# chaiyujin/sdfa-2019

Measured on AMD Instinct MI355X. Metric: animation frames/s/node (10 s@16 kHz clips); max|Δdgrad| vs CPU ref, higher is better.
Workload: dtype f32

## Files before the change

sdfa-2019_amd/csrc/api_core.cpp:

```cpp
#include "../../include/sdfa_stream.h"
#include "host.h"

#include <climits>
#include <cstdio>
#include <cstring>
#include <string>

static thread_local std::string g_err;

int sdfa_failv(int code, const char *fmt, va_list ap) {
    char buf[512];
    vsnprintf(buf, sizeof buf, fmt, ap);
    g_err = buf;
    return code;
}

int sdfa_fail(int code, const char *fmt, ...) {
    va_list ap;
    va_start(ap, fmt);
    sdfa_failv(code, fmt, ap);
    va_end(ap);
    return code;
}

thread_local int g_sdfa_mel_fft_radix4 = 0;
thread_local int g_sdfa_gather_plain_order = 0;
thread_local int g_sdfa_frontend_two_kernel = 0;
thread_local int g_sdfa_frontend_stream_block = 0;
thread_local int g_sdfa_frontend_stream_slots = 0;
thread_local int g_sdfa_frontend_stream_spin_max = 0;
thread_local int g_sdfa_frontend_stream_phases = 0;
thread_local int g_sdfa_frontend_t_major = 0;
extern thread_local int g_sdfa_gemm_variant;
thread_local int g_sdfa_freq_lstm_shape = 0;
thread_local int g_sdfa_pca_lds = 0;
thread_local int g_sdfa_pca_fp32 = 0;
thread_local int g_sdfa_conv_fp32 = 0;
thread_local int g_sdfa_time_lstm_split = 0;
thread_local int g_sdfa_time_lstm_handoff = 0;
thread_local int g_sdfa_time_lstm_timeout_us = 0;
thread_local int g_sdfa_share_gx0_off = 0;
thread_local int g_sdfa_encoder_dedup_off = 0;
thread_local int g_sdfa_freq_proj_tail = 0;
thread_local int g_sdfa_attn_unfused = 0;

extern "C" {

int sdfa_abi_version(void) { return SDFA_ABI_VERSION; }
int sdfa_stream_abi_version(void) { return SDFA_STREAM_ABI_VERSION; }
const char *sdfa_last_error(void) { return g_err.c_str(); }

int sdfa_debug_set_option(const char *name, int value) {
    struct Option { const char *name; int *var; int lo = INT_MIN, hi = INT_MAX; const char *accepts = nullptr; };
    thread_local const Option options[] = {
        {"attn_unfused", &g_sdfa_attn_unfused},
        {"share_gx0_off", &g_sdfa_share_gx0_off},
        {"encoder_dedup_off", &g_sdfa_encoder_dedup_off},
        {"freq_proj_tail", &g_sdfa_freq_proj_tail, 0, 2, "0 (rule), 1 (never) or 2 (always)"},
        {"frontend_two_kernel", &g_sdfa_frontend_two_kernel},
        {"frontend_stream_phases", &g_sdfa_frontend_stream_phases},
        {"frontend_stream_spin_max", &g_sdfa_frontend_stream_spin_max, 0, INT_MAX, "0 (default) or a positive poll count"},
        {"frontend_stream_block", &g_sdfa_frontend_stream_block, 0, 256, "0 (default) or 1..256 frames"},
        {"frontend_stream_slots", &g_sdfa_frontend_stream_slots, 0, 256, "0 (default) or 1..256 workgroups per block"},
        {"gather_plain_order", &g_sdfa_gather_plain_order},
        {"mel_fft_radix4", &g_sdfa_mel_fft_radix4},
        {"frontend_t_major", &g_sdfa_frontend_t_major},
        {"time_lstm_timeout_us", &g_sdfa_time_lstm_timeout_us},
        {"time_lstm_handoff", &g_sdfa_time_lstm_handoff},
        {"time_lstm_split", &g_sdfa_time_lstm_split},
        {"gemm_variant", &g_sdfa_gemm_variant},
        {"freq_lstm_shape", &g_sdfa_freq_lstm_shape},
        {"pca_lds", &g_sdfa_pca_lds},
        {"conv_fp32", &g_sdfa_conv_fp32},
        {"pca_fp32", &g_sdfa_pca_fp32},
    };
    for (const Option &o : options)
        if (name && !strcmp(name, o.name)) {
            if (value < o.lo || value > o.hi) return sdfa_fail(SDFA_EINVAL, "%s: %s", o.name, o.accepts);
            *o.var = value;
            return SDFA_OK;
        }
    return sdfa_fail(SDFA_EINVAL, "unknown option '%s'", name ? name : "(null)");
}

}
```

sdfa-2019_amd/csrc/api_forward.cpp:

```cpp
#include "common.h"
#include "host.h"
#include "kernels.h"
#include "model.h"

#include <algorithm>

extern thread_local int g_sdfa_gemm_variant, g_sdfa_freq_lstm_shape, g_sdfa_pca_lds, g_sdfa_pca_fp32, g_sdfa_conv_fp32, g_sdfa_share_gx0_off, g_sdfa_attn_unfused, g_sdfa_encoder_dedup_off,
    g_sdfa_freq_proj_tail;

namespace {

constexpr int64_t CT_WORDS = 2048, CT_FLAGS = 16, ST_WORDS = SDFA_WS_STATUS_BYTES / 4;

struct Ws {
    int64_t P1, X3, HF, Z, GX, H0, H1, KP, QC, QP, ZK, SH, ZU, total;
    int64_t TRUNK, A0, A1, COEF;
    int64_t CT_FREQ, CT_PCA, CT_FLAG;
};

Ws layout(int64_t Nc, bool keep) {
    const int64_t Mc = 64 * Nc;
    Ws w{};
    int64_t o = 0;
    auto take = [&](int64_t n) { int64_t r = o; o += round_up(n, 64); return r; };
    take(ST_WORDS);
    if (keep) {
        w.P1 = take(2048 * Mc); w.X3 = take(2048 * Mc); w.HF = take((int64_t)HF_SLAB_ROWS * 4 * Mc); w.Z = take(256 * Mc);
        w.GX = take(2048 * Mc); w.H0 = take(512 * Mc); w.H1 = take(512 * Mc); w.KP = take(128 * Mc);
    } else {
        const int64_t A = take(2048 * Mc);
        const int64_t B = take(2048 * Mc);
        w.HF = take((int64_t)HF_SLAB_ROWS * 4 * Mc);
        w.P1 = A; w.GX = A;
        w.X3 = B; w.Z = B; w.H0 = B + 256 * Mc; w.H1 = B + 768 * Mc; w.KP = B + 1280 * Mc;
    }
    w.QC = take(512 * Nc); w.QP = take(128 * Nc); w.ZK = take(512 * Nc);
    const int64_t R = take(2560 * Nc);
    w.TRUNK = R; w.A0 = R + 512 * Nc; w.A1 = R + 1024 * Nc; w.COEF = R + 1280 * Nc;
    w.SH = take(sdfa_share_table_words(Nc) + 111);
    w.ZU = keep ? take(256 * Mc) : w.P1;
    const int64_t CT = take(CT_WORDS);
    w.CT_FREQ = CT; w.CT_PCA = CT + 1; w.CT_FLAG = CT + CT_FLAGS;
    w.total = o;
    return w;
}

int64_t capacity(int64_t bytes, bool keep) {
    const int64_t per128 = layout(128, keep).total * 4;
    int64_t nc = (bytes / per128 + 2) * 128;
    while (nc > 0 && layout(nc, keep).total * 4 > bytes) nc -= 128;
    return nc;
}

struct Prof {
    const sdfa_model *m;
    hipStream_t s;
    hipEvent_t pending = nullptr;
    void begin(const char *stage) {
        if (!m->profile) return;
        sdfa_model::Ev e; e.stage = stage;
        (void)hipEventCreate(&e.a); (void)hipEventCreate(&e.b);
        (void)hipEventRecord(e.a, s);
        pending = e.b;
        std::lock_guard<std::mutex> lk(m->ev_mu);
        m->events.push_back(e);
    }
    void end() {
        if (!m->profile || !pending) return;
        (void)hipEventRecord(pending, s);
        pending = nullptr;
    }
};

GemmArgs gemm_fc(const sdfa_model::Fc &fc, const float *Q, int64_t ldq, float *D, int64_t Nc, const int64_t *spk, int64_t nreal) {
    GemmArgs g = sdfa_gemm_k4(fc.w, fc.Ppad, Q, ldq, D, Nc, fc.K);
    g.bias = fc.b; g.cond_w = fc.cw; g.cond_idx = fc.cw ? spk : nullptr;
    g.Pstore = fc.Pstore; g.Qreal = nreal; g.act = fc.act;
    return g;
}

}

extern "C" {

int64_t sdfa_workspace_bytes(const sdfa_model *m, int64_t max_frames) {
    if (!m || max_frames <= 0) return sdfa_fail(SDFA_EINVAL, "workspace_bytes: bad argument");
    return layout(round_up(max_frames, 128), m->keep).total * 4;
}

int sdfa_debug_keep_intermediates(sdfa_model *m, int on) {
    if (!m) return sdfa_fail(SDFA_EINVAL, "null model");
    m->keep = on != 0;
    return SDFA_OK;
}

int sdfa_profile_enable(sdfa_model *m, int on) {
    if (!m) return sdfa_fail(SDFA_EINVAL, "null model");
    std::lock_guard<std::mutex> lk(m->ev_mu);
    m->profile = on != 0;
    for (auto &e : m->events) { (void)hipEventDestroy(e.a); (void)hipEventDestroy(e.b); }
    m->events.clear();
    return SDFA_OK;
}

float sdfa_profile_ms(const sdfa_model *m, const char *stage) {
    if (!m || !stage) return (float)sdfa_fail(SDFA_EINVAL, "profile_ms: bad argument");
    float total = 0.f;
    bool any = false;
    std::lock_guard<std::mutex> lk(m->ev_mu);
    for (auto &e : m->events)
        if (e.stage == stage) {
            float ms = 0.f;
            if (hipEventSynchronize(e.b) != hipSuccess || hipEventElapsedTime(&ms, e.a, e.b) != hipSuccess)
                return (float)sdfa_fail(SDFA_EHIP, "profile_ms: event query failed");
            total += ms; any = true;
        }
    return any ? total : (float)sdfa_fail(SDFA_EINVAL, "profile_ms: no such stage '%s'", stage);
}

int sdfa_profile_reset(sdfa_model *m) { return m ? sdfa_profile_enable(m, m->profile) : sdfa_fail(SDFA_EINVAL, "null model"); }

enum { STAGE_BODY = 0, STAGE_ATTENTION = 1, STAGE_REGRESSOR = 2 };
static int stage_terms(const sdfa_model *m, int stage) {
    switch (m->precision) {
    case SDFA_PREC_BF16_ATTENTION: return stage == STAGE_ATTENTION ? 1 : 0;
    case SDFA_PREC_BF16X3_ATTENTION: return stage == STAGE_ATTENTION ? 3 : 0;
    case SDFA_PREC_BF16X6: return 6;
    case SDFA_PREC_BF16X3: return 3;
    case SDFA_PREC_BF16: return 1;
    default: return 0;
    }
}

int sdfa_model_set_precision(sdfa_model *m, int mode) {
    if (!m) return sdfa_fail(SDFA_EINVAL, "null model");
    if (mode < SDFA_PREC_FP32 || mode > SDFA_PREC_BF16X6) return sdfa_fail(SDFA_EINVAL, "unknown precision mode %d", mode);
    m->precision = mode;
    return SDFA_OK;
}

int sdfa_model_precision(const sdfa_model *m) { return m ? m->precision : SDFA_EINVAL; }

int sdfa_model_set_reserved_cus(sdfa_model *m, int k) {
    if (!m) return sdfa_fail(SDFA_EINVAL, "null model");
    if (k < 0 || k > 128) return sdfa_fail(SDFA_EINVAL, "reserved_cus must be in [0, 128], got %d", k);
    m->reserved_cus.store(k);
    return SDFA_OK;
}

static int encoder_impl(const sdfa_model *m, const float *d_audio_feat, int64_t n_frames, const int32_t *d_frame_clip,
                        const int64_t *d_frame_start, int hop, float *d_z, float *d_align, void *d_workspace,
                        int64_t workspace_bytes, void *stream) {
    if (!m || !m->finalized) return sdfa_fail(SDFA_ESTATE, "encoder_forward: model not finalised");
    if (n_frames == 0) return SDFA_OK;
    if (!d_audio_feat || !d_z || !d_workspace || n_frames < 0) return sdfa_fail(SDFA_EINVAL, "encoder_forward: bad argument");
    if (((uintptr_t)d_workspace | (uintptr_t)d_audio_feat | (uintptr_t)d_z) & 15) return sdfa_fail(SDFA_EINVAL, "encoder_forward: pointers must be 16-byte aligned");
    if ((uintptr_t)d_align & 3) return sdfa_fail(SDFA_EINVAL, "encoder_forward: d_align must be 4-byte aligned");
    const int64_t cap = capacity(workspace_bytes, m->keep);
    if (cap < 128) return sdfa_fail(SDFA_ENOSPACE, "encoder_forward: workspace of %lld bytes holds no 128-frame chunk", (long long)workspace_bytes);
    hipStream_t s = (hipStream_t)stream;
    Prof pf{m, s};
    float *ws = (float *)d_workspace;
    for (int64_t f0 = 0; f0 < n_frames; f0 += cap) {
        const int64_t N = std::min(cap, n_frames - f0);
        const int64_t Nc = round_up(N, 128), Mc = 64 * Nc;
        const Ws w = layout(Nc, m->keep);
        ConvArgs ca{};
        ca.audio_feat = d_audio_feat + f0 * (64 * 128 * 3); ca.N = N; ca.Nc = Nc; ca.Mc = Mc;
        ca.w1 = m->w1; ca.b1 = m->b1; ca.s1 = m->s1; ca.t1 = m->t1; ca.P1 = ws + w.P1;
        ca.w2 = m->w2; ca.b2 = m->b2; ca.s2 = m->s2; ca.t2 = m->t2;
        ca.w3 = m->w3; ca.b3 = m->b3; ca.s3 = m->s3; ca.t3 = m->t3; ca.X3 = ws + w.X3;
        const bool table = d_frame_clip != nullptr;
        const bool share = table || (!m->keep && !g_sdfa_encoder_dedup_off);
        const int64_t *d_ulimit = nullptr;
        int32_t *col_to_u = nullptr;
        bool split_tail = false;
        int64_t fat_grid = 0;
        const int64_t *d_qfull = nullptr;
        if (share) {
            ShareArgs sa{};
            sa.N = N; sa.Nc = Nc; sa.Mc = Mc;
            sdfa_share_carve(sa, reinterpret_cast<int32_t *>(ws + w.SH));
            split_tail = !m->keep && stage_terms(m, STAGE_BODY) == 0 && g_sdfa_gemm_variant == 0 && Mc / 256 >= 512 && g_sdfa_freq_proj_tail != 1;
            if (split_tail) {
                fat_grid = sdfa_fat_grid(256, Mc, sdfa_cu_count(), m->reserved_cus.load());
                sa.fat_grid = (int)fat_grid; sa.tail_mode = g_sdfa_freq_proj_tail;
            }
            pf.begin("share_map");
            if (table) {
                sa.frame_clip = d_frame_clip + f0; sa.frame_start = d_frame_start + f0; sa.hop = hop;
                sa.t_lo = 6; sa.t_hi = 58;
                HIP_TRY(sdfa_launch_share_map(sa, s));
            } else {
                sa.feat = ca.audio_feat;
                sa.hash = reinterpret_cast<uint64_t *>(ws + w.HF); sa.linked = sa.hash + Mc;
                HIP_TRY(sdfa_launch_share_map_content(sa, s));
            }
            pf.end();
            d_ulimit = sa.counts + 1; d_qfull = sa.counts + 2; col_to_u = sa.col_to_u;
            ca.col_src = sa.col_src; ca.col_limit = d_ulimit;
        }
        const int conv_terms = g_sdfa_conv_fp32 ? 0 : stage_terms(m, STAGE_BODY);
        if (m->keep && conv_terms) {
            pf.begin("conv1"); HIP_TRY(sdfa_launch_conv1(ca, s)); pf.end();
            ca.wb = m->cv_wb; ca.terms = conv_terms;
            pf.begin("conv23"); HIP_TRY(sdfa_launch_conv123(ca, s)); pf.end();
        } else if (m->keep) {
            pf.begin("conv1"); HIP_TRY(sdfa_launch_conv1(ca, s)); pf.end();
            pf.begin("conv23"); HIP_TRY(sdfa_launch_conv23(ca, s)); pf.end();
        } else {
            ca.wb = m->cv_wb; ca.terms = conv_terms;
            pf.begin("conv23"); HIP_TRY(sdfa_launch_conv123(ca, s)); pf.end();
        }

        const int fl_terms = stage_terms(m, STAGE_BODY);
        FreqLstmArgs fa{ws + w.X3, m->fl_w, m->fl_b, ws + w.HF, Mc, d_ulimit, m->fl_wb, fl_terms, reinterpret_cast<int *>(ws + w.CT_FREQ),
                        g_sdfa_freq_lstm_shape ? g_sdfa_freq_lstm_shape : (fl_terms ? 0 : m->freq_shape.load()), m->reserved_cus.load()};
        pf.begin("freq_lstm"); HIP_TRY(sdfa_launch_freq_lstm(fa, s)); pf.end();

        GemmArgs g = sdfa_gemm_k4(m->fp_w, 256, ws + w.HF, Mc, ws + w.Z, Mc, 8192);
        g.bias = m->fp_b; g.q_tile_major = 1; g.q_slab_rows = HF_SLAB_ROWS;
        g.terms = stage_terms(m, STAGE_BODY);
        g.reserve_cus = m->reserved_cus.load();
        if (share) { g.D = ws + w.ZU; g.q_limit = split_tail ? d_qfull : d_ulimit; }
        pf.begin("freq_proj");
        HIP_TRY(sdfa_launch_gemm(g, s));
        if (split_tail) {
            GemmTailArgs gt{m->fp_w, ws + w.HF, m->fp_b, ws + w.ZU, Mc, HF_SLAB_ROWS, d_qfull, d_ulimit, (int)fat_grid - 1};
            HIP_TRY(sdfa_launch_gemm_tail(gt, s));
        }
        pf.end();
        const bool share_gx0 = share && !m->keep && stage_terms(m, STAGE_BODY) == 0 && !g_sdfa_share_gx0_off;
        if (share && !share_gx0) {
            pf.begin("share_expand"); HIP_TRY(sdfa_launch_expand_cols(ws + w.ZU, col_to_u, ws + w.Z, 64, Mc, s)); pf.end();
        }

        const float *xin = share_gx0 ? ws + w.ZU : ws + w.Z;
        float *hout[2] = {ws + w.H0, ws + w.H1};
        const char *gxn[2] = {"gx0", "gx1"}, *lsn[2] = {"lstm0", "lstm1"};
        for (int l = 0; l < 2; ++l) {
            const bool mapped = share_gx0 && l == 0;
            float *gx = mapped ? ws + w.HF : ws + w.GX;
            GemmArgs gi = sdfa_gemm_k4(m->gx_w[l], 2048, xin, Mc, gx, Mc, l == 0 ? 256 : 512);
            gi.terms = stage_terms(m, STAGE_BODY);
            gi.reserve_cus = m->reserved_cus.load();
            if (mapped) gi.q_limit = d_ulimit;
            pf.begin(gxn[l]); HIP_TRY(sdfa_launch_gemm(gi, s)); pf.end();
            TimeLstmArgs ta{gx, m->tl_w[l], hout[l], Nc, Mc, m->tl_wb[l], stage_terms(m, STAGE_BODY),
                            reinterpret_cast<unsigned *>(ws + w.CT_FLAG), CT_WORDS - CT_FLAGS, m->tl_w16[l],
                            reinterpret_cast<unsigned *>(ws), m->reserved_cus.load(), mapped ? col_to_u : nullptr};
            pf.begin(lsn[l]); HIP_TRY(sdfa_launch_time_lstm(ta, s)); pf.end();
            xin = hout[l];
        }
        const int at_terms = stage_terms(m, STAGE_ATTENTION);
        const bool key_fused = g_sdfa_attn_unfused != 1;
        pf.begin("attn_proj");
        GemmArgs gk = sdfa_gemm_k4(m->kp_w, 128, ws + w.H1, Mc, ws + w.KP, Mc, 512);
        gk.terms = at_terms;
        if (!key_fused) HIP_TRY(sdfa_launch_gemm(gk, s));
        GemmArgs gc = sdfa_gemm_k4(m->qc_w, 512, ws + w.H1 + 31 * Nc * 4, Mc, ws + w.QC, Nc, 1536);
        gc.seg_k = 512; gc.seg_col = Nc; gc.terms = at_terms;
        HIP_TRY(sdfa_launch_gemm(gc, s));
        GemmArgs gq = sdfa_gemm_k4(m->qp_w, 128, ws + w.QC, Nc, ws + w.QP, Nc, 512);
        gq.terms = at_terms;
        HIP_TRY(sdfa_launch_gemm(gq, s));
        const bool tail_fused = key_fused && (at_terms == 0 || at_terms == 6) && g_sdfa_attn_unfused != 2 && sdfa_attn_fuses_tail(Nc, m->reserved_cus.load());
        if (key_fused) {
            AttnKeyArgs ak{};
            ak.Wk = m->kp_w; ak.H = ws + w.H1; ak.QP = ws + w.QP; ak.v = m->at_v; ak.b = m->at_b;
            ak.S = ws + w.KP;
            ak.Nc = Nc; ak.Mc = Mc; ak.terms = at_terms == 6 ? 0 : at_terms; ak.reserve_cus = m->reserved_cus.load();
            if (tail_fused) {
                ak.fuse_tail = 1; ak.Zk4 = ws + w.ZK; ak.z_out = d_z + f0 * 512; ak.align_out = d_align ? d_align + f0 * 64 : nullptr; ak.N = N;
            }
            HIP_TRY(sdfa_launch_attn_key_score(ak, s));
        }
        pf.end();

        AttnArgs aa{};
        aa.KP = ws + w.KP; aa.QP = ws + w.QP; aa.H = ws + w.H1; aa.v = m->at_v; aa.b = m->at_b;
        aa.Zk4 = ws + w.ZK; aa.z_out = d_z + f0 * 512; aa.align_out = d_align ? d_align + f0 * 64 : nullptr;
        aa.N = N; aa.Nc = Nc; aa.Mc = Mc;
        aa.S = key_fused ? ws + w.KP : nullptr;
        pf.begin("attn"); if (!tail_fused) HIP_TRY(sdfa_launch_attn(aa, s)); pf.end();
    }
    return SDFA_OK;
}

int sdfa_model_autotune(sdfa_model *m, int64_t n_frames, void *d_workspace, int64_t workspace_bytes, void *stream) {
    if (!m || !m->finalized) return sdfa_fail(SDFA_ESTATE, "autotune: model not finalised");
    if (!d_workspace || n_frames <= 0 || ((uintptr_t)d_workspace & 15)) return sdfa_fail(SDFA_EINVAL, "autotune: bad argument");
    const int64_t cap = capacity(workspace_bytes, m->keep);
    if (cap < 128) return sdfa_fail(SDFA_ENOSPACE, "autotune: workspace too small");
    const int64_t Nc = round_up(std::min(cap, n_frames), 128), Mc = 64 * Nc;
    const Ws w = layout(Nc, m->keep);
    float *ws = (float *)d_workspace;
    hipStream_t s = (hipStream_t)stream;
    HIP_TRY(hipMemsetAsync(ws + w.X3, 0, (size_t)2048 * Mc * sizeof(float), s));
    hipEvent_t e0, e1;
    HIP_TRY(hipEventCreate(&e0));
    HIP_TRY(hipEventCreate(&e1));
    static const int forms[] = {9, 8, 5, 3};
    float best_ms = 0.f;
    int best = m->freq_shape.load(), rc = SDFA_OK;
    for (int form : forms) {
        FreqLstmArgs fa{ws + w.X3, m->fl_w, m->fl_b, ws + w.HF, Mc, nullptr, m->fl_wb, 0, reinterpret_cast<int *>(ws + w.CT_FREQ), form, m->reserved_cus.load()};
        float ms = 0.f;
        for (int rep = 0; rep < 3 && rc == SDFA_OK; ++rep) {
            if (rep == 1 && hipEventRecord(e0, s) != hipSuccess) rc = SDFA_EHIP;
            if (sdfa_launch_freq_lstm(fa, s) != hipSuccess) rc = SDFA_EHIP;
        }
        if (rc == SDFA_OK && (hipEventRecord(e1, s) != hipSuccess || hipEventSynchronize(e1) != hipSuccess || hipEventElapsedTime(&ms, e0, e1) != hipSuccess)) rc = SDFA_EHIP;
        if (rc != SDFA_OK) break;
        if (best_ms == 0.f || ms < best_ms) { best_ms = ms; best = form; }
    }
    (void)hipEventDestroy(e0);
    (void)hipEventDestroy(e1);
    if (rc != SDFA_OK) return sdfa_fail(rc, "autotune: a HIP call failed: %s", hipGetErrorString(hipGetLastError()));
    m->freq_shape.store(best);
    return best;
}

int sdfa_encoder_forward(const sdfa_model *m, const float *d_audio_feat, int64_t n_frames, float *d_z, float *d_align,
                         void *d_workspace, int64_t workspace_bytes, void *stream) {
    return encoder_impl(m, d_audio_feat, n_frames, nullptr, nullptr, 0, d_z, d_align, d_workspace, workspace_bytes, stream);
}

int sdfa_encoder_forward_shared(const sdfa_model *m, const float *d_audio_feat, int64_t n_frames, const int32_t *d_frame_clip,
                                const int64_t *d_frame_start, int hop, float *d_z, float *d_align, void *d_workspace,
                                int64_t workspace_bytes, void *stream) {
    if (!d_frame_clip || !d_frame_start || hop <= 0) return sdfa_fail(SDFA_EINVAL, "encoder_forward_shared: frame table missing");
    return encoder_impl(m, d_audio_feat, n_frames, d_frame_clip, d_frame_start, hop, d_z, d_align, d_workspace, workspace_bytes, stream);
}

static hipError_t expand_rows(const sdfa_model *m, const float *coef, int64_t N, int64_t Nc, int64_t f0,
                              float *const *h_d_outs, int n_outs, int *queue, hipStream_t s) {
    float *d_out = h_d_outs[0];
    if (m->pca_n == 2) {
        PcaArgs pa{};
        pa.coef = coef; pa.basis_s = m->pca_q[0]; pa.basis_r = m->pca_q[1]; pa.mean_s = m->pca_bias[0]; pa.mean_r = m->pca_bias[1];
        pa.out = d_out + f0 * m->out_dim; pa.N = N; pa.Nc = Nc; pa.out_dim = m->out_dim;
        pa.n_extra = n_outs - 1;
        pa.reserve_cus = m->reserved_cus.load();
        pa.basis_b = m->pca_qb; pa.terms = (g_sdfa_pca_fp32 || m->precision != SDFA_PREC_BF16X3) ? 0 : 3;
        for (int x = 1; x < n_outs; ++x) pa.out_extra[x - 1] = h_d_outs[x] + f0 * m->out_dim;
        pa.ld_s = m->pca_ld[0]; pa.ld_r = m->pca_ld[1]; pa.cols_s = m->pca_cols[0]; pa.cols_r = m->pca_cols[1];
        if (g_sdfa_pca_lds != 4 && queue) return sdfa_launch_pca_dgrad_res(pa, queue, s);
        return sdfa_launch_pca_dgrad(pa, s);
// ... 159 lines not shown
```

sdfa-2019_amd/csrc/kernels.h:

```cpp
#pragma once
#include <hip/hip_runtime.h>
#include <stdint.h>

enum { ACT_NONE = 0, ACT_LRELU = 1, ACT_TANH = 2 };

constexpr int HF_SLAB_ROWS = 2048;
enum { OUT_K4 = 0, OUT_ROW = 1 };
constexpr int SDFA_MAX_DESTS = 8;

struct GemmArgs {
    const float *P;
    const float *Q;
    float *D;
    const float *bias;
    const float *cond_w;
    const int64_t *cond_idx;
    int64_t ldp, ldq, ldd;
    int64_t Ppad, Qpad;
    int64_t Pstore;
    int64_t Qreal;
    int K;
    int seg_k;
    int64_t seg_col;
    int act, out_mode, bias_on_q;
// ... 5 lines not shown
    float *D_extra[SDFA_MAX_DESTS - 1];
    int n_extra;
    int reserve_cus;
};
hipError_t sdfa_launch_gemm(const GemmArgs &a, hipStream_t s);
inline GemmArgs sdfa_gemm_k4(const float *P, int64_t rows, const float *Q, int64_t ldq, float *D, int64_t cols, int K) {
    GemmArgs g{};
    g.P = P; g.Q = Q; g.D = D;
    g.ldp = rows; g.Ppad = rows; g.Pstore = rows;
    g.ldq = ldq; g.ldd = cols; g.Qpad = cols; g.Qreal = cols;
    g.K = K; g.seg_k = K; g.act = ACT_NONE; g.out_mode = OUT_K4;
    return g;
}

struct PcaArgs {
    const float *coef;
    const float *basis_s, *basis_r;
    const float *mean_s, *mean_r;
    float *out;
    int64_t N, Nc, out_dim, ld_s, ld_r, cols_s, cols_r;
    float *out_extra[SDFA_MAX_DESTS - 1];
    int n_extra;
    int reserve_cus;
    const void *basis_b;
    int terms;
};
hipError_t sdfa_launch_pca_dgrad(const PcaArgs &a, hipStream_t s);
hipError_t sdfa_launch_pca_dgrad_res(const PcaArgs &a, int *queue, hipStream_t s);

struct FrontendConsts {
    const float *hamm;
    const float2 *twiddle;
    const int *mel_bin0;
    const float *mel_w8;
    int win, hop, sliding, nbins_used, nnz;
};
hipError_t sdfa_launch_frontend(const FrontendConsts &c, const float *pcm, const int64_t *clip_off,
                                const int64_t *clip_len, const int32_t *frame_clip, const int64_t *frame_start,
                                int64_t n_frames, float *audio_feat, hipStream_t s);
hipError_t sdfa_launch_mel_columns(const FrontendConsts &c, const float *pcm, const int64_t *clip_off, const int64_t *clip_len,
                                   const int32_t *frame_clip, const int64_t *frame_start, const int32_t *col_src,
                                   const int64_t *n_distinct, float *mel_table, hipStream_t s);
hipError_t sdfa_launch_mel_stream(const FrontendConsts &c, const float *pcm, const int64_t *clip_off, const int64_t *clip_len,
                                  const int32_t *frame_clip, const int64_t *frame_start, const int32_t *prev, const int32_t *shift,
                                  int64_t n_frames, int block, int slots, int producer_consumer, int spin_max, int *status, float *audio_feat, hipStream_t s);
hipError_t sdfa_launch_mel_ring(const FrontendConsts &c, const float *rings, int r, int n_rings, const int64_t *view_ring, const int64_t *view_hi,
                                const int32_t *frame_view, const int64_t *frame_start, const int32_t *prev, const int32_t *shift, int64_t n_frames,
                                int block, int slots, int producer_consumer, int spin_max, int *status, float *audio_feat, hipStream_t s);
hipError_t sdfa_launch_ring_append(float *rings, int r, int n_rings, const int64_t *seg, int n_seg, const float *src, int64_t n_src, hipStream_t s);
hipError_t sdfa_launch_gather_features(const float *mel_table, const int32_t *col_to_u, int64_t n_frames, int64_t Nc, int frame_major,
                                       float *audio_feat, hipStream_t s);

struct ConvArgs {
    const float *audio_feat;
    int64_t N, Nc, Mc;
    const float *w1, *b1, *s1, *t1;
    float *P1;
    const float *w2, *b2, *s2, *t2;
    const float *w3, *b3, *s3, *t3;
    float *X3;
    const int32_t *col_src;
    const int64_t *col_limit;
    const void *wb;
    int terms;
};
hipError_t sdfa_launch_conv1(const ConvArgs &a, hipStream_t s);
hipError_t sdfa_launch_conv23(const ConvArgs &a, hipStream_t s);
hipError_t sdfa_launch_conv123(const ConvArgs &a, hipStream_t s);

struct FreqLstmArgs {
    const float *X3;
    const float *W;
    const float *bias;
    float *HF;
    int64_t Mc;
    const int64_t *col_limit;
    const void *Wb;
    int terms;
    int *tile_counter;
    int shape;
    int reserve_cus;
};
hipError_t sdfa_launch_freq_lstm(const FreqLstmArgs &a, hipStream_t s);

struct TimeLstmArgs {
    const float *GX;
    const float *W;
    float *H;
    int64_t Nc, Mc;
    const void *Wb;
    int terms;
    unsigned *flags;
    int64_t flag_words;
    const float *W16;
    unsigned *status;
    int reserve_cus;
    const int32_t *col_map;
};
hipError_t sdfa_launch_time_lstm(const TimeLstmArgs &a, hipStream_t s);

struct AttnArgs {
    const float *KP;
    const float *QP;
    const float *H;
    const float *v;
    const float *b;
    float *Zk4;
    float *z_out;
    float *align_out;
    int64_t N, Nc, Mc;
    const float *S;
};
hipError_t sdfa_launch_attn(const AttnArgs &a, hipStream_t s);

struct AttnKeyArgs {
    const float *Wk;
    const float *H;
    const float *QP;
    const float *v, *b;
    float *S;
    int64_t Nc, Mc;
    int terms;
    int reserve_cus;
    int ts_shift;
    int fuse_tail;
    float *Zk4, *z_out, *align_out;
    int64_t N;
};
bool sdfa_attn_fuses_tail(int64_t Nc, int reserve_cus);
hipError_t sdfa_launch_attn_key_score(const AttnKeyArgs &a, hipStream_t s);

hipError_t sdfa_launch_rows_to_k4(const float *src, int64_t N, int F, float *dst, int64_t ld, hipStream_t s);
hipError_t sdfa_launch_rows_seg_to_k4(const float *src, int64_t src_ld, int64_t N, int c0, int nf, float *dst, int64_t ld,
                                      int f0, int nf_pad, hipStream_t s);
hipError_t sdfa_launch_k4_to_rows(const float *src, int64_t ld, int64_t N, int F, int f0, int nf, float *dst,
                                  int64_t dst_ld, hipStream_t s);
hipError_t sdfa_launch_tap(const float *src, int what, int64_t N, int64_t Nc, float *dst, hipStream_t s);

struct ShareArgs {
    const int32_t *frame_clip;
    const int64_t *frame_start;
    int hop;
    int t_lo, t_hi;
    int frame_major;
    int64_t N, Nc, Mc;
    int32_t *prev, *shift;
    int32_t *owner, *flag, *uid;
    int32_t *tile_sum;
    int32_t *col_src;
    int32_t *col_to_u;
    int64_t *counts;
    const float *feat;
    uint64_t *hash;
    uint64_t *linked;
    int fat_grid;
    int tail_mode;
};
inline int64_t sdfa_share_table_words(int64_t Nc) { return 16 + 2 * Nc + 5 * (64 * Nc) + (64 * Nc) / 1024 + 1; }
inline void sdfa_share_carve(ShareArgs &a, int32_t *base) {
    a.counts = reinterpret_cast<int64_t *>(base);
    a.prev = base + 16; a.shift = a.prev + a.Nc;
    a.owner = a.shift + a.Nc; a.flag = a.owner + a.Mc; a.uid = a.flag + a.Mc;
    a.col_src = a.uid + a.Mc; a.col_to_u = a.col_src + a.Mc; a.tile_sum = a.col_to_u + a.Mc;
}
hipError_t sdfa_launch_share_map(const ShareArgs &a, hipStream_t s);
hipError_t sdfa_launch_share_map_content(const ShareArgs &a, hipStream_t s);
hipError_t sdfa_launch_share_prev(const ShareArgs &a, hipStream_t s);
hipError_t sdfa_launch_expand_cols(const float *Zu, const int32_t *col_to_u, float *Z, int nquads, int64_t Mc, hipStream_t s);

struct GemmTailArgs {
    const float *P, *Q, *bias;
    float *D;
    int64_t ldd;
    int q_slab_rows;
    const int64_t *q_lo, *q_hi;
    int max_tiles;
};
hipError_t sdfa_launch_gemm_tail(const GemmTailArgs &a, hipStream_t s);
inline int64_t sdfa_fat_grid(int64_t rows, int64_t cols, int cus, int reserve_cus) {
    const int64_t ntiles = (rows / 256) * (cols / 256), wgs = cus - reserve_cus > 1 ? cus - reserve_cus : 1;
    return ntiles < wgs ? ntiles : wgs;
}

struct MeshArgs {
    const float *dgrad;
    int64_t n_frames;
    int n_tris, n_verts, n_free, free_pad;
    int n_src_tris;
    const int64_t *seek_src;
    const float *seek_w;
    const float *reg_xt;
    const int *inc_ptr;
    const int *inc_tri;
    const float *inc_coef;
    const int *vert_col;
    const float *tmpl;
    float *rhs;
    const float *sol;
    float *verts;
    int64_t ld;
};
hipError_t sdfa_launch_mesh_rhs(const MeshArgs &a, hipStream_t s);
hipError_t sdfa_launch_mesh_scatter(const MeshArgs &a, hipStream_t s);
hipError_t sdfa_launch_seek_plan(const int32_t *tslist, const int64_t *frame_off, const int64_t *query_off, int n_clips, double fps,
                                 int64_t n_queries, int64_t *src, float *w, hipStream_t s);
hipError_t sdfa_launch_seek_rows(const float *rows, int64_t width, const int64_t *src, const float *w, int64_t nq, float *out, hipStream_t s);
struct DgradArgs {
    const float *src;
    const float *target;
    const uint32_t *faces;
    const uint8_t *mask;
    int64_t n_frames;
    int n_tris, n_verts, target_is_offsets;
    double eps;
    float *out32;
    double *out64;
};
hipError_t sdfa_launch_deform_grad(const DgradArgs &a, hipStream_t s);
hipError_t sdfa_launch_ensemble_mean(const float *a, const float *b, int64_t n, float *out, hipStream_t s);

struct ResampleArgs {
    const float *x;
    int64_t n_in;
    float *y;
    int64_t n_res, n_out;
    const double *win, *delta;
    const double *treg;
    int64_t nwin, step;
    double scale;
    int num_table;
};
hipError_t sdfa_launch_resample(const ResampleArgs &a, hipStream_t s);
```

sdfa-2019_amd/csrc/share.hip:

```cpp
#include "common.h"
#include "kernels.h"

namespace {


__global__ void share_prev_kernel(ShareArgs a) {
    const int64_t n = (int64_t)blockIdx.x * blockDim.x + threadIdx.x;
    if (n >= a.Nc) return;
    int prev = -1, shift = 0;
    if (n < a.N) {
        const int clip = a.frame_clip[n];
        const int64_t s = a.frame_start[n];
        for (int back = 1; back <= 64 && n - back >= 0; ++back) {
            const int64_t q = n - back;
            if (a.frame_clip[q] != clip) break;
            const int64_t diff = s - a.frame_start[q];
            if (diff <= 0) break;
            if (diff > (int64_t)(a.t_hi - a.t_lo) * a.hop) break;
            if (diff % a.hop == 0) { prev = (int)q; shift = (int)(diff / a.hop); break; }
        }
    }
    a.prev[n] = prev;
    a.shift[n] = shift;
}

__device__ __forceinline__ int64_t col_index(const ShareArgs &a, int64_t n, int t) { return a.frame_major ? n * 64 + t : (int64_t)t * a.Nc + n; }
__device__ __forceinline__ void col_of(const ShareArgs &a, int64_t i, int64_t &n, int &t) {
    if (a.frame_major) { n = i >> 6; t = (int)(i & 63); } else { n = i % a.Nc; t = (int)(i / a.Nc); }
}

__global__ void share_owner_kernel(ShareArgs a) {
    const int64_t i = (int64_t)blockIdx.x * blockDim.x + threadIdx.x;
    if (i >= a.Mc) return;
    int64_t n;
    int t;
    col_of(a, i, n, t);
    if (n >= a.N) { a.owner[i] = -1; a.flag[i] = 0; return; }
    while (t >= a.t_lo && t <= a.t_hi) {
        const int p = a.prev[n];
        if (p < 0) break;
        const int tt = t + a.shift[n];
        if (tt > a.t_hi) break;
        n = p; t = tt;
    }
    const int64_t o = col_index(a, n, t);
    a.owner[i] = (int)o;
    a.flag[i] = o == i ? 1 : 0;
}

constexpr int COL_QUADS = 96;

__device__ __forceinline__ uint64_t mix64(uint64_t x) {
    x ^= x >> 32; x *= 0xd6e8feb86659fd93ull;
    x ^= x >> 32; x *= 0xd6e8feb86659fd93ull;
    return x ^ (x >> 32);
}

__global__ __launch_bounds__(256) void share_hash_kernel(ShareArgs a) {
    const int l = threadIdx.x & 31;
    const int64_t col = ((int64_t)blockIdx.x * 256 + threadIdx.x) >> 5, M = a.N * 64;
    uint64_t h = 0;
    if (col < M) {
        const uint4 *row = reinterpret_cast<const uint4 *>(a.feat) + col * COL_QUADS;
#pragma unroll
        for (int j = 0; j < 3; ++j) {
            const int q = l + 32 * j;
            const uint4 v = row[q];
            const uint64_t lo = (uint64_t)v.x | (uint64_t)v.y << 32, hi = (uint64_t)v.z | (uint64_t)v.w << 32;
            h += mix64(lo + 0x9e3779b97f4a7c15ull * (uint64_t)(2 * q + 1)) + mix64(hi + 0x9e3779b97f4a7c15ull * (uint64_t)(2 * q + 2));
        }
    }
    for (int off = 16; off; off >>= 1) h += __shfl_xor(h, off);
    if (col < M && l == 0) a.hash[col] = mix64(h) | 1;
}

constexpr int MATCH_SLOTS = 128;
__global__ __launch_bounds__(256) void share_match_kernel(ShareArgs a) {
    __shared__ unsigned long long hn[4][64], tab[4][MATCH_SLOTS];
    const int w = threadIdx.x >> 6, lane = threadIdx.x & 63;
    const int64_t n = (int64_t)blockIdx.x * 4 + w;
    const bool real = n < a.N && n > 0;
    const unsigned long long mine = real ? a.hash[n * 64 + lane] : 1;
    hn[w][lane] = mine;
    tab[w][lane] = 0; tab[w][lane + 64] = 0;
    __syncthreads();
    for (int slot = (int)(mine >> 8) & (MATCH_SLOTS - 1), k = 0; k < MATCH_SLOTS; ++k, slot = (slot + 1) & (MATCH_SLOTS - 1)) {
        const unsigned long long old = atomicCAS(&tab[w][slot], 0ull, mine);
        if (old == 0 || old == mine) break;
    }
    __syncthreads();
    if (n >= a.Nc) return;
    int best = 0, bp = -1, bd = 0;
    if (real) {
        const int64_t lo = n > 64 ? n - 64 : 0;
        unsigned long long hp = a.hash[(n - 1) * 64 + lane];
        for (int64_t p = n - 1; p >= lo && best < 63; --p) {
            const unsigned long long hq = p > lo ? a.hash[(p - 1) * 64 + lane] : 0;
            bool member = false;
            for (int slot = (int)(hp >> 8) & (MATCH_SLOTS - 1), k = 0; k < MATCH_SLOTS; ++k, slot = (slot + 1) & (MATCH_SLOTS - 1)) {
                const unsigned long long v = tab[w][slot];
                if (v == hp) member = true;
                if (v == hp || v == 0) break;
            }
            if (__ballot(member)) {
                for (int d0 = 1; d0 < 64 - best; d0 += 4) {
                    int c[4];
#pragma unroll
                    for (int k = 0; k < 4; ++k) {
                        const int d = d0 + k;
                        const bool eq = lane >= d && hn[w][lane >= d ? lane - d : 0] == hp;
                        c[k] = __popcll(__ballot(eq));
                    }
#pragma unroll
                    for (int k = 0; k < 4; ++k)
                        if (c[k] > best) { best = c[k]; bp = (int)p; bd = d0 + k; }
                }
            }
            hp = hq;
        }
    }
    if (lane == 0) { a.prev[n] = bp; a.shift[n] = bd; }
}

__global__ __launch_bounds__(256) void share_verify_kernel(ShareArgs a) {
    const int64_t n = blockIdx.x;
    const int w = threadIdx.x >> 6, lane = threadIdx.x & 63, half = lane >> 5, l = lane & 31;
    const int p = a.prev[n], d = a.shift[n];
    unsigned bits = 0;
    if (p >= 0) {
        const uint64_t *hn = a.hash + n * 64, *hp = a.hash + (int64_t)p * 64;
        const uint4 *fn = reinterpret_cast<const uint4 *>(a.feat) + n * 64 * COL_QUADS;
        const uint4 *fp = reinterpret_cast<const uint4 *>(a.feat) + (int64_t)p * 64 * COL_QUADS;
        for (int j = 0; j < 8; ++j) {
            const int t = 16 * w + 2 * j + half, tt = t + d;
            const bool cand = tt < 64 && hn[t] == hp[tt];
            bool differ = false;
            if (cand) {
#pragma unroll
                for (int k = 0; k < 3; ++k) {
                    const uint4 x = fn[t * COL_QUADS + l + 32 * k], y = fp[tt * COL_QUADS + l + 32 * k];
                    differ |= ((x.x ^ y.x) | (x.y ^ y.y) | (x.z ^ y.z) | (x.w ^ y.w)) != 0;
                }
            }
            const uint64_t c = __ballot(cand), bad = __ballot(differ);
            if ((c & 1) && !(bad & 0xffffffffull)) bits |= 1u << (2 * j);
            if ((c >> 32 & 1) && !(bad >> 32)) bits |= 1u << (2 * j + 1);
        }
    }
    if (lane == 0) reinterpret_cast<uint16_t *>(a.linked)[n * 4 + w] = (uint16_t)bits;
}

__global__ void share_owner_content_kernel(ShareArgs a) {
    const int64_t i = (int64_t)blockIdx.x * blockDim.x + threadIdx.x;
    if (i >= a.Mc) return;
    int64_t n;
    int t;
    col_of(a, i, n, t);
    if (n >= a.N) { a.owner[i] = -1; a.flag[i] = 0; return; }
    while (t < 63 && (a.linked[n] >> t & 1)) {
        t += a.shift[n];
        n = a.prev[n];
    }
    const int64_t o = col_index(a, n, t);
    a.owner[i] = (int)o;
    a.flag[i] = o == i ? 1 : 0;
}

__device__ __forceinline__ int block_inclusive_scan_1024(int v, int *part) {
    const int tid = threadIdx.x;
    part[tid] = v;
    __syncthreads();
    for (int off = 1; off < 1024; off <<= 1) {
        const int x = tid >= off ? part[tid - off] : 0;
        __syncthreads();
        part[tid] += x;
        __syncthreads();
    }
    return part[tid];
}

__global__ __launch_bounds__(1024) void share_scan_tiles_kernel(ShareArgs a) {
    __shared__ int part[1024];
    const int64_t i = (int64_t)blockIdx.x * 1024 + threadIdx.x;
    const int f = i < a.Mc ? a.flag[i] : 0;
    const int inc = block_inclusive_scan_1024(f, part);
    if (i < a.Mc) a.uid[i] = inc - f;
    if (threadIdx.x == 1023) a.tile_sum[blockIdx.x] = inc;
}

constexpr int TAIL_NUM = 3, TAIL_DEN = 4;
__global__ __launch_bounds__(1024) void share_scan_sums_kernel(ShareArgs a, int ntiles) {
    __shared__ int part[1024];
    int carry = 0;
    for (int base = 0; base < ntiles; base += 1024) {
        const int t = base + threadIdx.x;
        const int v = t < ntiles ? a.tile_sum[t] : 0;
        const int inc = block_inclusive_scan_1024(v, part);
        if (t < ntiles) a.tile_sum[t] = carry + inc - v;
        carry += part[1023];
        __syncthreads();
    }
    if (threadIdx.x == 0) {
        const int64_t mu = carry, pad = (mu + 255) / 256 * 256;
        a.counts[0] = mu;
        a.counts[1] = pad;
        int64_t q_full = pad;
        if (a.fat_grid > 0 && a.tail_mode != 1) {
            const int64_t T = pad / 256, G = a.fat_grid, r = T % G;
            if (a.tail_mode == 2 || r * TAIL_DEN <= G * TAIL_NUM) q_full = (T - r) * 256;
        }
        a.counts[2] = q_full;
    }
}

__global__ __launch_bounds__(1024) void share_scan_fix_kernel(ShareArgs a) {
    const int64_t i = (int64_t)blockIdx.x * 1024 + threadIdx.x;
    const int64_t mu = a.counts[0], pad = a.counts[1];
    if (i < a.Mc) {
        const int u = a.uid[i] + a.tile_sum[blockIdx.x];
        a.uid[i] = u;
        int64_t n;
        int t;
        col_of(a, i, n, t);
        if (a.flag[i]) a.col_src[u] = (int)(n * 64 + t);
    }
    if (i >= mu && i < pad) a.col_src[i] = -1;
}

__global__ void share_assign_kernel(ShareArgs a) {
    const int64_t m = (int64_t)blockIdx.x * blockDim.x + threadIdx.x;
    if (m >= a.Mc) return;
    const int o = a.owner[m];
    a.col_to_u[m] = o >= 0 ? a.uid[o] : 0;
}

__global__ void expand_cols_kernel(const float4 *__restrict__ Zu, const int32_t *__restrict__ col_to_u, float4 *__restrict__ Z,
                                   int nquads, int64_t Mc) {
    const int64_t m = (int64_t)blockIdx.x * blockDim.x + threadIdx.x;
    if (m >= Mc) return;
    const int64_t u = col_to_u[m];
    for (int q = 0; q < nquads; ++q) Z[(int64_t)q * Mc + m] = Zu[(int64_t)q * Mc + u];
}

}

static void launch_share_numbering(const ShareArgs &a, hipStream_t s) {
    const int ntiles = (int)((a.Mc + 1023) / 1024);
    hipLaunchKernelGGL(share_scan_tiles_kernel, dim3(ntiles), dim3(1024), 0, s, a);
    hipLaunchKernelGGL(share_scan_sums_kernel, dim3(1), dim3(1024), 0, s, a, ntiles);
    hipLaunchKernelGGL(share_scan_fix_kernel, dim3(ntiles), dim3(1024), 0, s, a);
    hipLaunchKernelGGL(share_assign_kernel, dim3((unsigned)((a.Mc + 255) / 256)), dim3(256), 0, s, a);
}

hipError_t sdfa_launch_share_map_content(const ShareArgs &a, hipStream_t s) {
    hipLaunchKernelGGL(share_hash_kernel, dim3((unsigned)(a.N * 8)), dim3(256), 0, s, a);
    hipLaunchKernelGGL(share_match_kernel, dim3((unsigned)(a.Nc / 4)), dim3(256), 0, s, a);
    hipLaunchKernelGGL(share_verify_kernel, dim3((unsigned)a.N), dim3(256), 0, s, a);
    hipLaunchKernelGGL(share_owner_content_kernel, dim3((unsigned)((a.Mc + 255) / 256)), dim3(256), 0, s, a);
    launch_share_numbering(a, s);
    return hipGetLastError();
}

hipError_t sdfa_launch_share_map(const ShareArgs &a, hipStream_t s) {
    hipLaunchKernelGGL(share_prev_kernel, dim3((unsigned)((a.Nc + 255) / 256)), dim3(256), 0, s, a);
    hipLaunchKernelGGL(share_owner_kernel, dim3((unsigned)((a.Mc + 255) / 256)), dim3(256), 0, s, a);
    launch_share_numbering(a, s);
    return hipGetLastError();
}

hipError_t sdfa_launch_share_prev(const ShareArgs &a, hipStream_t s) {
    hipLaunchKernelGGL(share_prev_kernel, dim3((unsigned)((a.Nc + 255) / 256)), dim3(256), 0, s, a);
    return hipGetLastError();
}

hipError_t sdfa_launch_expand_cols(const float *Zu, const int32_t *col_to_u, float *Z, int nquads, int64_t Mc, hipStream_t s) {
    hipLaunchKernelGGL(expand_cols_kernel, dim3((unsigned)((Mc + 255) / 256)), dim3(256), 0, s,
                       reinterpret_cast<const float4 *>(Zu), col_to_u, reinterpret_cast<float4 *>(Z), nquads, Mc);
    return hipGetLastError();
}
```

Baseline: 144,000.

## Replace windowed chain matching with a global hash table for content-based column sharing

The content-based sharing map now inserts each column's hash into a global open-addressed table that keeps the minimum column index per hash. A single resolve kernel then looks up the group owner and verifies the feature bytes. This replaces the per-window match kernel, the verify kernel and the chain-following owner kernel. It removes the 64-frame search window and pointer chasing, so duplicates can be found across the whole batch. In exchange it adds a memset of the table and global atomics, and columns whose hash collides but whose content differs fall back to owning themselves. A debug option that truncates the hash bits is added.

```diff
diff --git a/sdfa-2019_amd/csrc/api_core.cpp b/sdfa-2019_amd/csrc/api_core.cpp
--- a/sdfa-2019_amd/csrc/api_core.cpp
+++ b/sdfa-2019_amd/csrc/api_core.cpp
@@ -41,6 +41,7 @@
 thread_local int g_sdfa_time_lstm_timeout_us = 0;
 thread_local int g_sdfa_share_gx0_off = 0;
 thread_local int g_sdfa_encoder_dedup_off = 0;
+thread_local int g_sdfa_share_hash_bits = 0;
 thread_local int g_sdfa_freq_proj_tail = 0;
 thread_local int g_sdfa_attn_unfused = 0;
 
@@ -56,6 +57,7 @@
         {"attn_unfused", &g_sdfa_attn_unfused},
         {"share_gx0_off", &g_sdfa_share_gx0_off},
         {"encoder_dedup_off", &g_sdfa_encoder_dedup_off},
+        {"share_hash_bits", &g_sdfa_share_hash_bits, 0, 32, "0 (the whole hash) or 1..32 low bits"},
         {"freq_proj_tail", &g_sdfa_freq_proj_tail, 0, 2, "0 (rule), 1 (never) or 2 (always)"},
         {"frontend_two_kernel", &g_sdfa_frontend_two_kernel},
         {"frontend_stream_phases", &g_sdfa_frontend_stream_phases},
diff --git a/sdfa-2019_amd/csrc/api_forward.cpp b/sdfa-2019_amd/csrc/api_forward.cpp
--- a/sdfa-2019_amd/csrc/api_forward.cpp
+++ b/sdfa-2019_amd/csrc/api_forward.cpp
@@ -6,7 +6,7 @@
 #include <algorithm>
 
 extern thread_local int g_sdfa_gemm_variant, g_sdfa_freq_lstm_shape, g_sdfa_pca_lds, g_sdfa_pca_fp32, g_sdfa_conv_fp32, g_sdfa_share_gx0_off, g_sdfa_attn_unfused, g_sdfa_encoder_dedup_off,
-    g_sdfa_freq_proj_tail;
+    g_sdfa_freq_proj_tail, g_sdfa_share_hash_bits;
 
 namespace {
 
@@ -193,7 +193,10 @@
                 HIP_TRY(sdfa_launch_share_map(sa, s));
             } else {
                 sa.feat = ca.audio_feat;
-                sa.hash = reinterpret_cast<uint64_t *>(ws + w.HF); sa.linked = sa.hash + Mc;
+                sa.hash = reinterpret_cast<uint64_t *>(ws + w.HF);
+                sa.group_slots = sdfa_share_group_slots(N);
+                sa.group_key = sa.hash + Mc; sa.group_first = reinterpret_cast<uint32_t *>(sa.group_key + sa.group_slots);
+                sa.hash_bits = g_sdfa_share_hash_bits;
                 HIP_TRY(sdfa_launch_share_map_content(sa, s));
             }
             pf.end();
diff --git a/sdfa-2019_amd/csrc/kernels.h b/sdfa-2019_amd/csrc/kernels.h
--- a/sdfa-2019_amd/csrc/kernels.h
+++ b/sdfa-2019_amd/csrc/kernels.h
@@ -181,11 +181,15 @@
     int64_t *counts;
     const float *feat;
     uint64_t *hash;
-    uint64_t *linked;
+    uint64_t *group_key;
+    uint32_t *group_first;
+    int64_t group_slots;
+    int hash_bits;
     int fat_grid;
     int tail_mode;
 };
 inline int64_t sdfa_share_table_words(int64_t Nc) { return 16 + 2 * Nc + 5 * (64 * Nc) + (64 * Nc) / 1024 + 1; }
+inline int64_t sdfa_share_group_slots(int64_t N) { int64_t s = 1024; while (s < 2 * 64 * N) s <<= 1; return s; }
 inline void sdfa_share_carve(ShareArgs &a, int32_t *base) {
     a.counts = reinterpret_cast<int64_t *>(base);
     a.prev = base + 16; a.shift = a.prev + a.Nc;
diff --git a/sdfa-2019_amd/csrc/share.hip b/sdfa-2019_amd/csrc/share.hip
--- a/sdfa-2019_amd/csrc/share.hip
+++ b/sdfa-2019_amd/csrc/share.hip
@@ -49,6 +49,7 @@
 }
 
 constexpr int COL_QUADS = 96;
+constexpr unsigned long long GROUP_EMPTY = ~0ull;
 
 __device__ __forceinline__ uint64_t mix64(uint64_t x) {
     x ^= x >> 32; x *= 0xd6e8feb86659fd93ull;
@@ -71,99 +72,62 @@
         }
     }
     for (int off = 16; off; off >>= 1) h += __shfl_xor(h, off);
-    if (col < M && l == 0) a.hash[col] = mix64(h) | 1;
-}
-
-constexpr int MATCH_SLOTS = 128;
-__global__ __launch_bounds__(256) void share_match_kernel(ShareArgs a) {
-    __shared__ unsigned long long hn[4][64], tab[4][MATCH_SLOTS];
-    const int w = threadIdx.x >> 6, lane = threadIdx.x & 63;
-    const int64_t n = (int64_t)blockIdx.x * 4 + w;
-    const bool real = n < a.N && n > 0;
-    const unsigned long long mine = real ? a.hash[n * 64 + lane] : 1;
-    hn[w][lane] = mine;
-    tab[w][lane] = 0; tab[w][lane + 64] = 0;
+    h = mix64(h);
+    if (a.hash_bits) h &= (1ull << a.hash_bits) - 1;
+    h |= 1;
+    __shared__ unsigned long long wg_hash[8];
+    const int c = threadIdx.x >> 5;
+    if (l == 0) { a.hash[col] = h; wg_hash[c] = h; }
     __syncthreads();
-    for (int slot = (int)(mine >> 8) & (MATCH_SLOTS - 1), k = 0; k < MATCH_SLOTS; ++k, slot = (slot + 1) & (MATCH_SLOTS - 1)) {
-        const unsigned long long old = atomicCAS(&tab[w][slot], 0ull, mine);
-        if (old == 0 || old == mine) break;
-    }
-    __syncthreads();
-    if (n >= a.Nc) return;
-    int best = 0, bp = -1, bd = 0;
-    if (real) {
-        const int64_t lo = n > 64 ? n - 64 : 0;
-        unsigned long long hp = a.hash[(n - 1) * 64 + lane];
-        for (int64_t p = n - 1; p >= lo && best < 63; --p) {
-            const unsigned long long hq = p > lo ? a.hash[(p - 1) * 64 + lane] : 0;
-            bool member = false;
-            for (int slot = (int)(hp >> 8) & (MATCH_SLOTS - 1), k = 0; k < MATCH_SLOTS; ++k, slot = (slot + 1) & (MATCH_SLOTS - 1)) {
-                const unsigned long long v = tab[w][slot];
-                if (v == hp) member = true;
-                if (v == hp || v == 0) break;
-            }
-            if (__ballot(member)) {
-                for (int d0 = 1; d0 < 64 - best; d0 += 4) {
-                    int c[4];
+    if (l) return;
+    for (int j = 0; j < c; ++j)
+        if (wg_hash[j] == h) return;
+    const unsigned long long key = ~h;
+    const unsigned i = (unsigned)col_index(a, col >> 6, (int)(col & 63));
+    unsigned long long *keys = reinterpret_cast<unsigned long long *>(a.group_key);
+    const int64_t mask = a.group_slots - 1;
+    for (int64_t slot = (int64_t)(h >> 1) & mask, k = 0; k <= mask; ++k, slot = (slot + 1) & mask) {
+        unsigned long long cur = __hip_atomic_load(&keys[slot], __ATOMIC_RELAXED, __HIP_MEMORY_SCOPE_AGENT);
+        if (cur == GROUP_EMPTY) {
+            cur = atomicCAS(&keys[slot], GROUP_EMPTY, key);
+            if (cur == GROUP_EMPTY) cur = key;
+        }
+        if (cur != key) continue;
+        if (__hip_atomic_load(&a.group_first[slot], __ATOMIC_RELAXED, __HIP_MEMORY_SCOPE_AGENT) > i) atomicMin(&a.group_first[slot], i);
+        break;
+    }
+}
+
+__global__ __launch_bounds__(256) void share_resolve_kernel(ShareArgs a) {
+    const int l = threadIdx.x & 31, half = (threadIdx.x & 63) >> 5;
+    const int64_t col = ((int64_t)blockIdx.x * 256 + threadIdx.x) >> 5, n = col >> 6;
+    const int64_t i = col_index(a, n, (int)(col & 63));
+    if (n >= a.N) {
+        if (l == 0) { a.owner[i] = -1; a.flag[i] = 0; }
+        return;
+    }
+    const uint64_t h = a.hash[col], mask = (uint64_t)a.group_slots - 1;
+    uint64_t slot = (h >> 1) & mask;
+    for (uint64_t k = 0; k < mask && a.group_key[slot] != ~h; ++k) slot = (slot + 1) & mask;
+    const int64_t cand = a.group_key[slot] == ~h ? (int64_t)a.group_first[slot] : i;
+    bool differ = false;
+    if (cand != i) {
+        int64_t cn;
+        int ct;
+        col_of(a, cand, cn, ct);
+        const uint4 *x = reinterpret_cast<const uint4 *>(a.feat) + col * COL_QUADS, *y = reinterpret_cast<const uint4 *>(a.feat) + (cn * 64 + ct) * COL_QUADS;
 #pragma unroll
-                    for (int k = 0; k < 4; ++k) {
-                        const int d = d0 + k;
-                        const bool eq = lane >= d && hn[w][lane >= d ? lane - d : 0] == hp;
-                        c[k] = __popcll(__ballot(eq));
-                    }
-#pragma unroll
-                    for (int k = 0; k < 4; ++k)
-                        if (c[k] > best) { best = c[k]; bp = (int)p; bd = d0 + k; }
-                }
-            }
-            hp = hq;
-        }
-    }
-    if (lane == 0) { a.prev[n] = bp; a.shift[n] = bd; }
-}
-
-__global__ __launch_bounds__(256) void share_verify_kernel(ShareArgs a) {
-    const int64_t n = blockIdx.x;
-    const int w = threadIdx.x >> 6, lane = threadIdx.x & 63, half = lane >> 5, l = lane & 31;
-    const int p = a.prev[n], d = a.shift[n];
-    unsigned bits = 0;
-    if (p >= 0) {
-        const uint64_t *hn = a.hash + n * 64, *hp = a.hash + (int64_t)p * 64;
-        const uint4 *fn = reinterpret_cast<const uint4 *>(a.feat) + n * 64 * COL_QUADS;
-        const uint4 *fp = reinterpret_cast<const uint4 *>(a.feat) + (int64_t)p * 64 * COL_QUADS;
-        for (int j = 0; j < 8; ++j) {
-            const int t = 16 * w + 2 * j + half, tt = t + d;
-            const bool cand = tt < 64 && hn[t] == hp[tt];
-            bool differ = false;
-            if (cand) {
-#pragma unroll
-                for (int k = 0; k < 3; ++k) {
-                    const uint4 x = fn[t * COL_QUADS + l + 32 * k], y = fp[tt * COL_QUADS + l + 32 * k];
-                    differ |= ((x.x ^ y.x) | (x.y ^ y.y) | (x.z ^ y.z) | (x.w ^ y.w)) != 0;
-                }
-            }
-            const uint64_t c = __ballot(cand), bad = __ballot(differ);
-            if ((c & 1) && !(bad & 0xffffffffull)) bits |= 1u << (2 * j);
-            if ((c >> 32 & 1) && !(bad >> 32)) bits |= 1u << (2 * j + 1);
-        }
-    }
-    if (lane == 0) reinterpret_cast<uint16_t *>(a.linked)[n * 4 + w] = (uint16_t)bits;
-}
-
-__global__ void share_owner_content_kernel(ShareArgs a) {
-    const int64_t i = (int64_t)blockIdx.x * blockDim.x + threadIdx.x;
-    if (i >= a.Mc) return;
-    int64_t n;
-    int t;
-    col_of(a, i, n, t);
-    if (n >= a.N) { a.owner[i] = -1; a.flag[i] = 0; return; }
-    while (t < 63 && (a.linked[n] >> t & 1)) {
-        t += a.shift[n];
-        n = a.prev[n];
-    }
-    const int64_t o = col_index(a, n, t);
-    a.owner[i] = (int)o;
-    a.flag[i] = o == i ? 1 : 0;
+        for (int k = 0; k < 3; ++k) {
+            const uint4 u = x[l + 32 * k], v = y[l + 32 * k];
+            differ |= ((u.x ^ v.x) | (u.y ^ v.y) | (u.z ^ v.z) | (u.w ^ v.w)) != 0;
+        }
+    }
+    const uint64_t bad = __ballot(differ) >> (32 * half) & 0xffffffffull;
+    if (l == 0) {
+        const int64_t o = bad ? i : cand;
+        a.owner[i] = (int)o;
+        a.flag[i] = o == i ? 1 : 0;
+    }
 }
 
 __device__ __forceinline__ int block_inclusive_scan_1024(int v, int *part) {
@@ -253,10 +217,10 @@
 }
 
 hipError_t sdfa_launch_share_map_content(const ShareArgs &a, hipStream_t s) {
+    const hipError_t e = hipMemsetAsync(a.group_key, 0xff, (size_t)a.group_slots * 12, s);
+    if (e != hipSuccess) return e;
     hipLaunchKernelGGL(share_hash_kernel, dim3((unsigned)(a.N * 8)), dim3(256), 0, s, a);
-    hipLaunchKernelGGL(share_match_kernel, dim3((unsigned)(a.Nc / 4)), dim3(256), 0, s, a);
-    hipLaunchKernelGGL(share_verify_kernel, dim3((unsigned)a.N), dim3(256), 0, s, a);
-    hipLaunchKernelGGL(share_owner_content_kernel, dim3((unsigned)((a.Mc + 255) / 256)), dim3(256), 0, s, a);
+    hipLaunchKernelGGL(share_resolve_kernel, dim3((unsigned)(a.Nc * 8)), dim3(256), 0, s, a);
     launch_share_numbering(a, s);
     return hipGetLastError();
 }
```

After: 148,800 (median of 6 runs). 1.03x the previous value.
